# quanpn90/avsr

Measured on AMD Instinct MI355X. Metric: AV-frames/sec/GPU (fwd+bwd) on 15s clips; WER parity on LRS2 test, higher is better.
Workload: dtype bf16

## Files before the change

### avsr_amd/_lib.py

```python
import ctypes
import os

import torch

_HERE = os.path.dirname(os.path.abspath(__file__))
LIB_PATH = os.environ.get("AVSR_LIB_PATH_AB") or os.path.join(_HERE, "libavsr_hip.so")

AVSR_F32, AVSR_BF16 = 0, 1
ACT_NONE, ACT_GELU, ACT_RELU = 0, 1, 2

_c_p = ctypes.c_void_p
_i64 = ctypes.c_int64
_f = ctypes.c_float
_i = ctypes.c_int


class GemmParams(ctypes.Structure):
    _fields_ = [
        ("M", _i), ("N", _i), ("K", _i), ("batch", _i),
        ("dtype", _i), ("a_kmajor", _i), ("b_kmajor", _i), ("c_f32", _i),
        ("A", _c_p), ("lda", _i64), ("strideA", _i64),
        ("B", _c_p), ("ldb", _i64), ("strideB", _i64),
        ("C", _c_p), ("ldc", _i64), ("strideC", _i64),
        ("alpha", _f), ("beta", _f),
# ... 240 lines not shown
    _fields_ = [("B", _i), ("L", _i), ("x", _c_p), ("ldx", _i64), ("noise", _c_p), ("ldn", _i64),
                ("lengths", _c_p), ("snr_db", _c_p), ("y", _c_p), ("ldy", _i64), ("ws", _c_p)]


class VideoNormParams(ctypes.Structure):
    _fields_ = [
        ("B", _i), ("T", _i), ("H", _i), ("W", _i), ("crop", _i), ("oy", _i), ("ox", _i),
        ("frames", _c_p), ("mean", _f), ("std", _f), ("out", _c_p),
    ]


SYMBOLS = {
    "avsr_version": ([], ctypes.c_char_p),
    "avsr_set_option": ([_i, _i64], _i),
    "avsr_get_option": ([_i], _i64),
    "avsr_gemm": ([ctypes.POINTER(GemmParams), _c_p], _i),
    "avsr_gemm_wgrad_group": ([ctypes.POINTER(GemmParams), _i, _c_p], _i),
    "avsr_gemm_skinny_splits": ([_i, _i, _i], _i),
    "avsr_conv_fwd": ([ctypes.POINTER(ConvParams), _c_p], _i),
    "avsr_conv_bwd_data": ([ctypes.POINTER(ConvParams), _c_p], _i),
    "avsr_conv_bwd_weight": ([ctypes.POINTER(ConvParams), _c_p], _i),
    "avsr_conv_stat_tiles": ([ctypes.POINTER(ConvParams)], _i),
    "avsr_conv_bnr_tiles": ([ctypes.POINTER(ConvParams)], _i),
    "avsr_conv_wgrad_ws": ([ctypes.POINTER(ConvParams)], _i64),
    "avsr_conv_path": ([ctypes.POINTER(ConvParams), _i], _i),
    "avsr_layernorm_fwd": ([ctypes.POINTER(LayerNormParams), _c_p], _i),
    "avsr_layernorm_bwd": ([ctypes.POINTER(LayerNormParams), _c_p], _i),
    "avsr_bn_finalize": ([ctypes.POINTER(BnFinalizeParams), _c_p], _i),
    "avsr_bn_act_fwd": ([ctypes.POINTER(BnActParams), _c_p], _i),
    "avsr_bn_act_bwd_reduce": ([ctypes.POINTER(BnActParams), _c_p], _i),
    "avsr_bn_bwd_apply": ([ctypes.POINTER(BnActParams), _c_p], _i),
    "avsr_stem_pool_fwd": ([ctypes.POINTER(StemPoolParams), _c_p], _i),
    "avsr_stem_pool_bwd_apply": ([ctypes.POINTER(StemPoolParams), _c_p], _i),
    "avsr_bn_bwd_finalize": ([ctypes.POINTER(BnActParams), _i, _c_p], _i),
    "avsr_avgpool_fwd": ([_i, _i, _i, _i, _c_p, _c_p, _c_p], _i),
    "avsr_avgpool_bwd": ([_i, _i, _i, _i, _c_p, _c_p, _c_p], _i),
    "avsr_attn_fwd": ([ctypes.POINTER(AttnParams), _c_p], _i),
    "avsr_debug_attn_stamps": ([_c_p], _i),
    "avsr_attn_bwd_prep": ([ctypes.POINTER(AttnParams), _c_p], _i),
    "avsr_attn_bwd": ([ctypes.POINTER(AttnParams), _c_p], _i),
    "avsr_attn_dropmask": ([ctypes.POINTER(AttnParams), _c_p], _i),
    "avsr_attn_path": ([ctypes.POINTER(AttnParams), _i], _i),
    "avsr_row_lse": ([ctypes.POINTER(XentParams), _c_p], _i),
    "avsr_lsm_fwd": ([ctypes.POINTER(XentParams), _c_p], _i),
    "avsr_lsm_bwd": ([ctypes.POINTER(XentParams), _c_p], _i),
    "avsr_ctc_fwd": ([ctypes.POINTER(CtcParams), _c_p], _i),
    "avsr_ctc_bwd": ([ctypes.POINTER(CtcParams), _c_p], _i),
    "avsr_ctc_align": ([ctypes.POINTER(CtcAlignParams), _c_p], _i),
    "avsr_ctc_beam": ([ctypes.POINTER(CtcBeamParams), _c_p], _i),
    "avsr_loss_finalize": ([_i, _c_p, _i, _c_p, _c_p, _f, _i, _c_p, _c_p], _i),
    "avsr_ew_bwd": ([ctypes.POINTER(EwParams), _c_p], _i),
    "avsr_colsum_defer": ([_i], _i),
    "avsr_colsum_flush": ([_c_p], _i),
    "avsr_colsum_inline": ([_i], _i),
    "avsr_dropout_fwd": ([ctypes.POINTER(EwParams), _c_p], _i),
    "avsr_mask_rows": ([_i, _i, _i, _i, _c_p, _i64, _c_p, _c_p], _i),
    "avsr_embed_fwd": ([ctypes.POINTER(EmbedParams), _c_p], _i),
    "avsr_embed_bwd": ([ctypes.POINTER(EmbedParams), _c_p], _i),
    "avsr_cast": ([_i, _i, _i, _i, _c_p, _i64, _c_p, _i64, _f, _f, _c_p], _i),
    "avsr_cast_flat": ([_i, _i, _i64, _c_p, _c_p, _c_p], _i),
    "avsr_stem_pack": ([_i, _i, _i, _c_p, _c_p, _c_p], _i),
    "avsr_stem_wpack": ([_i, _c_p, _c_p, _c_p], _i),
    "avsr_stem_conv_tiles": ([_i, _i], _i),
    "avsr_stem_wpack2": ([_c_p, _c_p, _c_p], _i),
    "avsr_stem_conv_fwd": ([_i, _i, _c_p, _c_p, _c_p, _c_p, _c_p], _i),
    "avsr_stem_wgrad_unpack": ([_c_p, _c_p, _c_p], _i),
# ... 24 lines not shown
}

_lib = None


class AvsrLibError(RuntimeError):
    pass


def load():
    global _lib
    if _lib is not None:
        return _lib
    if not os.path.exists(LIB_PATH):
        raise AvsrLibError(f"{LIB_PATH} not built: run `python -c 'import __graft_entry__ as g; g.build()'`")
    lib = ctypes.CDLL(LIB_PATH, mode=ctypes.RTLD_GLOBAL)
    for name, (argtypes, restype) in SYMBOLS.items():
        if os.environ.get("AVSR_LIB_PATH_AB") and not hasattr(lib, name):
            continue
        fn = getattr(lib, name)
        fn.argtypes = argtypes
        fn.restype = restype
    _lib = lib
    return lib


def check(rc, op):
    if rc != 0:
        raise AvsrLibError(f"{op} failed with code {rc}")


OPTIONS = {"gemm_tile": 0, "attn_sq_fwd": 1, "attn_sq_bwd": 2, "wgrad_dual": 3, "conv_192": 4, "conv_s2phase": 5,
           "conv_patch": 6, "conv_wpatch": 7, "stem_pool_2x2": 8,
           "stem_wpatch": 9, "attn_enc_fused": 10}
TILES = ["128", "256", "256x128", "128x256", "128s3", "128w8s3", "pp", "192", "192x256", "192w8s3", "64", "64s4"]
ATTN_PATHS = ["f32", "tiled", "resident", "sq", "enc"]
CONV_PATHS = ["reg", "glds", "patch", "s2", "wpatch", "stem_wpatch"]
CONV_PASSES = ["fwd", "dgrad", "wgrad"]


def set_option(name, value):
    if name == "gemm_tile" and not isinstance(value, int):
        value = 0 if value in (None, "auto") else TILES.index(value) + 1
    lib = load()
    prev = get_option(name)
    check(lib.avsr_set_option(OPTIONS[name], int(value)), f"avsr_set_option({name}, {value})")
    return prev


def get_option(name):
    return int(load().avsr_get_option(OPTIONS[name]))


_raw_stream = getattr(torch._C, "_cuda_getCurrentRawStream", None)
_get_device = getattr(torch._C, "_cuda_getDevice", None) or torch.cuda.current_device


def stream_ptr(device=None):
    if _raw_stream is not None:
        idx = _get_device() if device is None else torch.device(device).index
        if idx is None:
            idx = _get_device()
        return ctypes.c_void_p(_raw_stream(idx))
    return ctypes.c_void_p(torch.cuda.current_stream(device).cuda_stream)
```

### avsr_amd/csrc/conv.h

```cpp
#pragma once
#include "gemm_core.h"
#include "gemm_glds.h"

namespace conv {
using namespace gemmcore;
using gemmg::GBK;
using gemmg::OOB;
using gemmg::bglds16;
using gemmg::make_rsrc;

struct ConvArgs {
  ConvGeom g;
  uint32_t a_bytes, b_bytes;
  const void* a; const void* b;
  int64_t a_gstride, b_gstride, c_gstride;
  int M, N, K, splits, kchunk;
  float* ws;
  Epi e;
  gemmg::BnrArgs bnr;
};

enum { K_FWD = 0, K_DGRAD = 1, K_WGRAD = 2, K_DGRAD_BNR = 3 };

struct WgradPlan { int splits, kchunk; bool slab; };
// ... 11 lines not shown

template <int R, int NW> struct BWgtR {
  static constexpr bool KMAJ = false;
  static constexpr int CPR = R / 8, RPP = 64 / CPR, SLOTS = GBK / RPP / NW;
  __amdgpu_buffer_rsrc_t rs; ConvGeom g;
  uint32_t vo[SLOTS];
  AVSR_DEV void init(const bf16* base, uint32_t bytes, const ConvGeom& g_, int r0, int rext, int wave, int lane) {
    rs = make_rsrc(base, bytes); g = g_;
    const int ktot = g.ktot_w;
#pragma unroll
    for (int i = 0; i < SLOTS; ++i) {
      const int pc = i * NW + wave, pk = pc * RPP + lane / CPR;
      const int r = r0 + ((lane % CPR) ^ gemmg::rswz<CPR>(pk)) * 8;
      vo[i] = r < rext ? (uint32_t)(((int64_t)pk * ktot + r) * 2) : OOB;
    }
  }
  AVSR_DEV void issue(char* img, int k0, int wave) const {
    const int ktot = g.ktot_w;
    int tap = k0 >> g.cout_shift;
    if (g.tap_step != 1) {
      const int u = (int)fdiv(tap, g.f_kw), v = tap - u * (int)g.f_kw.d;
      tap = (g.tap_kh0 + g.tap_step * u) * g.tap_kfw + g.tap_kw0 + g.tap_step * v;
    }
    const uint32_t so = (uint32_t)((((int64_t)(k0 & ((1 << g.cout_shift) - 1))) * ktot + (int64_t)tap * g.cin) * 2);
#pragma unroll
    for (int i = 0; i < SLOTS; ++i) bglds16(rs, vo[i], so, img + (i * NW + wave) * 1024);
  }
};

int igemm_f32(int kind, int bm, const ConvArgs& a, int groups, hipStream_t st);
int igemm_glds(int kind, int bm, const ConvArgs& a, int groups, hipStream_t st);
int patch_launch(int kind, const ConvArgs& a, const avsr_conv_params* p, hipStream_t st);
int wpatch_launch(const avsr_conv_params* p, hipStream_t st);
int stem_wpatch_launch(const avsr_conv_params* p, hipStream_t st);
int wgrad_reduce(float* ws, int splits, int chunks, int64_t mn, int groups, float* dw, int64_t dw_gstride, hipStream_t st);
}
```

### avsr_amd/csrc/conv.hip

```cpp
#include "conv.h"

namespace conv {
namespace {

int ilog2(int v) { int s = 0; while ((1 << s) < v) ++s; return (1 << s) == v ? s : -1; }

int make_geom(const avsr_conv_params* p, ConvGeom& g) {
  g.nimg = p->nimg; g.hin = p->hin; g.win = p->win; g.hout = p->hout; g.wout = p->wout;
  g.kh = p->kh; g.kw = p->kw; g.sh = p->sh; g.sw = p->sw; g.ph = p->ph; g.pw = p->pw;
  g.cin = p->cin; g.cout = p->cout; g.ldx = p->ldx; g.ldy = p->ldy;
  g.f_hw_out = make_fastdiv((uint32_t)(p->hout * p->wout));
  g.f_w_out = make_fastdiv((uint32_t)p->wout);
  g.f_hw_in = make_fastdiv((uint32_t)(p->hin * p->win));
  g.f_w_in = make_fastdiv((uint32_t)p->win);
  g.f_kw = make_fastdiv((uint32_t)p->kw);
  g.cin_shift = ilog2(p->cin); g.cout_shift = ilog2(p->cout);
  g.ktot_w = p->kh * p->kw * p->cin; g.tap_kfw = p->kw; g.tap_kh0 = 0; g.tap_kw0 = 0; g.tap_step = 1;
  const int ve = p->dtype == AVSR_BF16 ? 8 : 4;
  if (g.cin_shift < 0 || g.cout_shift < 0 || p->cin < ve || p->cout < ve) return AVSR_E_SHAPE;
  if (p->ldx % ve || p->ldy % ve) return AVSR_E_ALIGN;
  if (p->groups < 1 || p->ldx < (int64_t)p->groups * p->cin || p->ldy < (int64_t)p->groups * p->cout) return AVSR_E_SHAPE;
  return 0;
}

// ... 275 lines not shown
    a.bnr.scale = p->bnr_scale; a.bnr.shift = p->bnr_shift; a.bnr.prelu = p->bnr_prelu;
    a.bnr.mean = p->bnr_mean; a.bnr.invstd = p->bnr_invstd; a.bnr.scale2 = p->bnr_scale2;
    a.bnr.shift2 = p->bnr_shift2; a.bnr.mean2 = p->bnr_mean2; a.bnr.invstd2 = p->bnr_invstd2; a.bnr.ws = p->bnr_ws;
    kind = K_DGRAD_BNR + (p->bnr_scale2 ? 2 : p->bnr_res ? 1 : 0);
  }
  if (a.M == 0) return 0;
  ConvPlan pl;
  if ((rc = conv_plan(p, AVSR_CONV_DGRAD, pl))) return rc;
  a.a_bytes = pl.a_bytes; a.b_bytes = pl.b_bytes;
  hipStream_t st = (hipStream_t)stream;
  switch (pl.path) {
    case AVSR_CONV_PATH_REG: return igemm_f32(kind, pl.bm, a, p->groups, st);
    case AVSR_CONV_PATH_S2: return s2_launch(kind, a, p, pl, st);
    case AVSR_CONV_PATH_PATCH: return patch_launch(kind, a, p, st);
    default: return igemm_glds(kind, pl.bm, a, p->groups, st);
  }
}

extern "C" int avsr_conv_bwd_weight(const avsr_conv_params* p, void* stream) {
  if (!p) return AVSR_E_ARG;
  ConvArgs a{};
  int rc = make_geom(p, a.g);
  if (rc) return rc;
  if (!avsr_aligned16(p->x) || !avsr_aligned16(p->dy) || !p->dw) return AVSR_E_ALIGN;
  a.a = p->dy; a.b = p->x;
  const int64_t ktot = (int64_t)p->kh * p->kw * p->cin;
  a.a_gstride = p->cout; a.b_gstride = p->cin; a.c_gstride = p->cout * ktot;
  a.M = p->cout; a.N = (int)ktot; a.K = p->nimg * p->hout * p->wout;
  if (a.K == 0) return 0;
  ConvPlan pl;
  if ((rc = conv_plan(p, AVSR_CONV_WGRAD, pl))) return rc;
  hipStream_t st = (hipStream_t)stream;
  if (pl.path == AVSR_CONV_PATH_WPATCH) return wpatch_launch(p, st);
  if (pl.path == AVSR_CONV_PATH_STEM_WPATCH) return stem_wpatch_launch(p, st);
  const WgradPlan& w = pl.w;
  a.a_bytes = pl.a_bytes; a.b_bytes = pl.b_bytes;
  a.splits = w.splits; a.kchunk = w.kchunk;
  a.ws = w.slab ? p->ws : nullptr;
  a.e.M = a.M; a.e.N = a.N; a.e.C = p->dw; a.e.ldc = ktot; a.e.alpha = 1.f;
  if (w.slab) { a.e.ldc = a.N; }
  else if (w.splits == 1) { a.e.beta = 1.f; }
  else { a.e.atomic = 1; }
  rc = pl.path == AVSR_CONV_PATH_REG ? igemm_f32(K_WGRAD, pl.bm, a, p->groups, st) : igemm_glds(K_WGRAD, pl.bm, a, p->groups, st);
  if (rc || !w.slab) return rc;
  const int64_t mn = (int64_t)a.M * a.N;
  const int64_t xb = (int64_t)avsr_grid(mn / 4, 256, 1024) * p->groups;
  int chunks = (int)((65536 / 256 + xb - 1) / xb);
  if (chunks > w.splits) chunks = w.splits;
  if (chunks < 1) chunks = 1;
  return wgrad_reduce(p->ws, w.splits, chunks, mn, p->groups, p->dw, a.c_gstride, st);
}
```

### avsr_amd/csrc/conv_wpatch.hip

```cpp
#include "conv.h"

namespace conv {
namespace {

template <int W_, int TR_, int TPI_, int NBUF_, int PST_, int IPT_ = 1, int NBLK_ = WP_BLOCKS, int SPREAD_ = 0>
struct WPGeo {
  static constexpr int W = W_, TR = TR_, TPI = TPI_, H = TR * TPI, NBUF = NBUF_, PST = PST_, IPT = IPT_, NBLK = NBLK_;
  static constexpr int IMGT = TR * W;
  static constexpr int PX = IPT * IMGT;
  static constexpr int KS = (PX + 31) / 32;
  static constexpr int DYR = KS * 32;
  static constexpr int WP = W + 2, PROWS = (IPT * (TR + 1) + 1) * WP;
  static constexpr int SLOTS = PST / 16;
  static constexpr int PPIECE = (PROWS * SLOTS + 255) / 256;
  static constexpr int PBYTES = PPIECE * 4 * 1024;
  static constexpr int DYPIECE = DYR * 128 / 4096;
  static constexpr int DYB = DYR * 128;
  static constexpr int BUF = DYB + PBYTES;
  static constexpr int LDS = NBUF * BUF;
  static constexpr int NP = DYPIECE + PPIECE;
  static constexpr int SPREAD = SPREAD_ > 0 ? SPREAD_ : KS;
  static_assert(LDS <= 160 * 1024, "the tile buffers must fit the CU's LDS");
  static_assert(IPT == 1 || TPI == 1, "a tile is part of one image or whole images");
  static_assert(NBUF >= 2 && (NBUF - 2) * NP <= 63 && SPREAD <= KS, "vmcnt range / DMA spread");
// ... 186 lines not shown
}

template <class G>
int wpatch_launch_g(const avsr_conv_params* p, hipStream_t st) {
  static bool attr = false;
  if (!attr) {
    (void)hipFuncSetAttribute((const void*)conv_wgrad_patch_kernel<G>, hipFuncAttributeMaxDynamicSharedMemorySize, G::LDS);
    attr = true;
  }
  const uint32_t bytes = (uint32_t)((int64_t)p->nimg * p->hin * p->win * p->cin * 2);
  const int nq = (p->cout / 64) * (p->cin / 64), S = G::NBLK / 8;
  if (nq <= S ? S % nq != 0 : (nq % S != 0 || 8 % (nq / S) != 0)) return AVSR_E_SHAPE;
  hipLaunchKernelGGL((conv_wgrad_patch_kernel<G>), dim3(G::NBLK), dim3(256), G::LDS, st, (const bf16*)p->x,
                     (const bf16*)p->dy, bytes, bytes, p->nimg, p->cin, p->cout, p->ws);
  AVSR_CHECK_LAUNCH();
  const unsigned gx = (64 * WP_COLS / 4 + 255) / 256;
  hipLaunchKernelGGL(wpatch_reduce_kernel, dim3(gx, (unsigned)nq, (unsigned)WPR_CHUNKS), dim3(256), 0, st, p->ws,
                     G::NBLK, p->cin, p->cout, p->dw, 0);
  AVSR_CHECK_LAUNCH();
  hipLaunchKernelGGL(wpatch_reduce_kernel, dim3(gx, (unsigned)nq, 1u), dim3(256), 0, st, p->ws, G::NBLK, p->cin,
                     p->cout, p->dw, 1);
  AVSR_CHECK_LAUNCH();
  return 0;
}

constexpr int SWP_TR = 4, SWP_TC = 48, SWP_KS = SWP_TC / 8, SWP_TPI = 44 / SWP_TR;
constexpr int SWP_DYB = SWP_KS * 32 * 128, SWP_DYPIECE = SWP_DYB / 4096;
constexpr int SWP_PR = 2 * SWP_TR + 5, SWP_PC = 103, SWP_SLOTS = SWP_PR * SWP_PC, SWP_RB = SWP_PC * 16;
constexpr int SWP_PPIECE = (SWP_SLOTS + 255) / 256, SWP_PBYTES = SWP_PPIECE * 4096;
constexpr int SWP_BUF = SWP_DYB + SWP_PBYTES, SWP_NBUF = 3, SWP_LDS = SWP_NBUF * SWP_BUF;
constexpr int SWP_NP = SWP_DYPIECE + SWP_PPIECE, SWP_PAIRS = 25;
constexpr int SWP_JW = (SWP_PAIRS + 3) / 4;
static_assert(SWP_LDS <= 160 * 1024 && SWP_DYB % 4096 == 0 && SWP_KS % 2 == 0, "stem weight-grad tile buffers");
static_assert(2 * (SWP_TC - 1) + 6 - 3 < SWP_PC - 3 + 1 && SWP_NP % SWP_KS == 0, "patch width / DMA spread");

AVSR_DEV int swp_toff(int t) {
  t = t > 48 ? 48 : t;
  const int kh = t / 7, kw = t - 7 * kh;
  return kh * SWP_RB + kw * 16;
}

__global__ __launch_bounds__(256, 1) void stem_wgrad_patch_kernel(const bf16* __restrict__ xp, const bf16* __restrict__ dy,
                                                                  uint32_t x_bytes, uint32_t dy_bytes, int nimg,
                                                                  float* __restrict__ ws) {
  extern __shared__ __attribute__((aligned(16))) char smem[];
  const int lane = threadIdx.x & 63, wave = __builtin_amdgcn_readfirstlane(threadIdx.x >> 6);
  const int ntiles = nimg * SWP_TPI;
  const int ta = (int)((int64_t)ntiles * blockIdx.x / gridDim.x), tb = (int)((int64_t)ntiles * (blockIdx.x + 1) / gridDim.x);
  const __amdgpu_buffer_rsrc_t rx = make_rsrc(xp, x_bytes), rdy = make_rsrc(dy, dy_bytes);
  uint32_t vdy[SWP_DYPIECE];
  int vpt[SWP_PPIECE], ppr[SWP_PPIECE];
#pragma unroll
  for (int i = 0; i < SWP_DYPIECE; ++i) {
    const int sl = (wave + 4 * i) * 64 + lane, row = sl >> 3;
    const int ch = (sl & 7) ^ whswz(row), k = row & 31, col = 8 * (row >> 5) + (k & 7);
    vdy[i] = col < 44 ? (uint32_t)(((k >> 3) * 44 + col) * 128 + ch * 16) : gemmg::OOB;
  }
#pragma unroll
  for (int i = 0; i < SWP_PPIECE; ++i) {
    const int sl = (wave + 4 * i) * 64 + lane, pr = sl / SWP_PC, pc = sl - pr * SWP_PC;
    const bool ok = sl < SWP_SLOTS && pc >= 3 && pc < 91;
    vpt[i] = ((pr - 3) * 88 + pc - 3) * 16;
    ppr[i] = ok ? pr - 3 : -1000;
  }
  auto issue = [&](int pc, int t, char* buf) {
    const int img = t / SWP_TPI, oy0 = (t - img * SWP_TPI) * SWP_TR;
    if (pc < SWP_DYPIECE) {
      gemmg::bglds16(rdy, vdy[pc], (uint32_t)(img * 1936 + oy0 * 44) * 128u, buf + (wave + 4 * pc) * 1024);
    } else {
      const int i = pc - SWP_DYPIECE, y = 2 * oy0 + ppr[i];
      const uint32_t vo = (uint32_t)y < 88u ? (uint32_t)(img * 123904 + oy0 * 2816 + vpt[i]) : gemmg::OOB;
      gemmg::bglds16(rx, vo, 0u, buf + SWP_DYB + (wave + 4 * i) * 1024);
    }
  };
  const int g = lane >> 4, qq = (lane & 15) >> 2, pp = lane & 3;
  const int pxa = 16 * (g >> 1) + 4 * (g & 1) + qq;
  const int sw = whswz(pxa);
  int dA[4];
#pragma unroll
  for (int i = 0; i < 4; ++i) dA[i] = pxa * 128 + (((2 * i + (pp >> 1)) ^ sw) << 4) + 8 * (pp & 1);
  const int pbase = SWP_DYB + (2 * (pxa >> 3) * SWP_PC + 2 * (pxa & 7)) * 16;
  int oB[SWP_JW];
#pragma unroll
  for (int j = 0; j < SWP_JW; ++j) oB[j] = pbase + swp_toff(2 * (wave + 4 * j) + (pp >> 1)) + 8 * (pp & 1);
  f32x4 acc[4][SWP_JW];
#pragma unroll
  for (int i = 0; i < 4; ++i)
#pragma unroll
    for (int j = 0; j < SWP_JW; ++j) acc[i][j] = f32x4{0.f, 0.f, 0.f, 0.f};
  constexpr int PD = SWP_NBUF - 1, PER = SWP_NP / SWP_KS;
#pragma unroll
  for (int d = 0; d < PD; ++d)
    if (ta + d < tb)
#pragma unroll
      for (int pc = 0; pc < SWP_NP; ++pc) issue(pc, ta + d, smem + d * SWP_BUF);
  struct Fr { bf16x8 a[4], b[SWP_JW]; };
  auto load = [&](Fr& f, const char* buf, int kb) {
#pragma unroll
    for (int i = 0; i < 4; ++i) f.a[i] = trpair(buf + dA[i] + kb * 4096, buf + dA[i] + kb * 4096 + 1024);
#pragma unroll
    for (int j = 0; j < SWP_JW; ++j) f.b[j] = trpair(buf + oB[j] + kb * 256, buf + oB[j] + kb * 256 + 2 * SWP_RB);
  };
  auto mma = [&](const Fr& f, int h) {
#pragma unroll
    for (int i = 2 * h; i < 2 * h + 2; ++i)
#pragma unroll
      for (int j = 0; j < SWP_JW; ++j) acc[i][j] = mfma16(f.a[i], f.b[j], acc[i][j]);
  };
  for (int t = ta; t < tb; ++t) {
    const char* buf = smem + ((t - ta) % SWP_NBUF) * SWP_BUF;
    char* nbuf = smem + ((t + PD - ta) % SWP_NBUF) * SWP_BUF;
    const bool more = t + PD < tb;
    if (t + 1 < tb) gemmg::wait_vmcnt<SWP_NP>();
    else gemmg::wait_vmcnt<0>();
    __builtin_amdgcn_s_barrier();
    asm volatile("" ::: "memory");
    Fr f0, f1;
    load(f0, buf, 0);
#pragma unroll
    for (int kb = 0; kb < SWP_KS; kb += 2) {
      mma(f0, 0);
      __builtin_amdgcn_sched_barrier(0);
      load(f1, buf, kb + 1);
      __builtin_amdgcn_sched_barrier(0);
      mma(f0, 1);
      if (more)
#pragma unroll
        for (int d = 0; d < PER; ++d) issue(kb * PER + d, t + PD, nbuf);
      mma(f1, 0);
      __builtin_amdgcn_sched_barrier(0);
      if (kb + 2 < SWP_KS) load(f0, buf, kb + 2);
      __builtin_amdgcn_sched_barrier(0);
      mma(f1, 1);
      if (more)
#pragma unroll
        for (int d = 0; d < PER; ++d) issue((kb + 1) * PER + d, t + PD, nbuf);
    }
  }
  float* o = ws + (int64_t)blockIdx.x * 64 * SWP_COLS;
#pragma unroll
  for (int j = 0; j < SWP_JW; ++j) {
    const int col = 16 * (wave + 4 * j) + (lane & 15);
    if (col < SWP_COLS)
#pragma unroll
      for (int i = 0; i < 4; ++i)
#pragma unroll
        for (int r = 0; r < 4; ++r) o[(16 * i + 4 * g + r) * SWP_COLS + col] = acc[i][j][r];
  }
}

}

int wpatch_launch(const avsr_conv_params* p, hipStream_t st) {
  if (p->cin == 64) return wpatch_launch_g<WPStage1>(p, st);
  if (p->cin == 128) return wpatch_launch_g<WPStage2>(p, st);
  if (p->cin == 256) return wpatch_launch_g<WPStage3>(p, st);
  return wpatch_launch_g<WPStage4>(p, st);
}

int stem_wpatch_launch(const avsr_conv_params* p, hipStream_t st) {
  static bool attr = false;
  if (!attr) {
    (void)hipFuncSetAttribute((const void*)stem_wgrad_patch_kernel, hipFuncAttributeMaxDynamicSharedMemorySize, SWP_LDS);
    attr = true;
  }
  const uint32_t xb = (uint32_t)((int64_t)p->nimg * 88 * 88 * 16), dyb = (uint32_t)((int64_t)p->nimg * 1936 * 128);
  hipLaunchKernelGGL(stem_wgrad_patch_kernel, dim3(SWP_BLOCKS), dim3(256), SWP_LDS, st, (const bf16*)p->x,
                     (const bf16*)p->dy, xb, dyb, p->nimg, p->ws);
  AVSR_CHECK_LAUNCH();
  return wgrad_reduce(p->ws, SWP_BLOCKS, 8, 64 * SWP_COLS, 1, p->dw, 0, st);
}
}
```

### avsr_amd/csrc/version.hip

```cpp
#include <atomic>

#include "common.h"

extern "C" const char* avsr_version(void) { return "avsr_hip 0.2.0 gfx950"; }

#ifndef AVSR_AB_ATTN_ENC_FUSED
#define AVSR_AB_ATTN_ENC_FUSED 1
#endif

namespace {
std::atomic<int64_t> g_opt[AVSR_OPT_COUNT] = {{0}, {1}, {0}, {1}, {1}, {1}, {1}, {1}, {1}, {1}, {AVSR_AB_ATTN_ENC_FUSED}};

bool opt_valid(int option, int64_t v) {
  switch (option) {
    case AVSR_OPT_GEMM_TILE: return v >= 0 && v <= AVSR_TILE_COUNT;
    case AVSR_OPT_ATTN_SQ_BWD: return v == 0;
    case AVSR_OPT_ATTN_SQ_FWD:
    case AVSR_OPT_WGRAD_DUAL:
    case AVSR_OPT_CONV_192:
    case AVSR_OPT_CONV_S2PHASE:
    case AVSR_OPT_CONV_PATCH:
    case AVSR_OPT_CONV_WPATCH:
    case AVSR_OPT_STEM_POOL_2X2:
    case AVSR_OPT_STEM_WPATCH:
    case AVSR_OPT_ATTN_ENC_FUSED: return v == 0 || v == 1;
    default: return false;
  }
}
}

int64_t avsr_opt(int option) { return g_opt[option].load(std::memory_order_relaxed); }

extern "C" int avsr_set_option(int option, int64_t value) {
  if (!opt_valid(option, value)) return AVSR_E_ARG;
  g_opt[option].store(value, std::memory_order_relaxed);
  return 0;
}

extern "C" int64_t avsr_get_option(int option) {
  if (option < 0 || option >= AVSR_OPT_COUNT) return -1;
  return avsr_opt(option);
}
```

### avsr_amd/engine.py

```python
import math
import os
import random

import numpy as np
import torch

from . import ops
from . import _lib as L
from .arena import Arena

GELU, RELU, NONE = L.ACT_GELU, L.ACT_RELU, L.ACT_NONE
_BN_FUSE = True
_DB_FUSE = True
_COLSUM_DEFER = True
_SIDE_BIAS = True
WGRAD_GROUP = False
SIDE_ORDER = "o,f2,f1,c,q"
ATTN_MASK = True
_CTC_SIDE = True
_STEM_DIRECT = True
_LN_EW_FUSE = True
SIDE_STREAM = True
EARLY_NORM = True
OPT_OVERLAP = True
# ... 544 lines not shown
                dz1, sums1 = da1, ops.bn_bwd_finalize(ws, tiles, cout, **g1)
            else:
                ops.conv_bwd_data(blk["g2"], dh2, self.w(p + "conv2.weight"), da1)
                dz1, sums1 = ops.bn_act_bwd_reduce(da1, blk["h1"], blk["st1"], prelu1, **g1)
            dh1 = self._e(M2, cout)
            ops.bn_bwd_apply(dz1, blk["h1"], blk["st1"], sums1, dh1)
            if self._live(p + "conv1.weight"):
                self._conv_wgrad(blk["g1"], blk["x"], dh1, self.g(p + "conv1.weight"))
            if fuse:
                if j > 0:
                    pb = blocks[j - 1]
                    pdown = pb["gd"] is not None
                    tgt = dict(h=pb["h2"], st=pb["st2"], prelu=self.arena.master(pb["p"] + "relu2.weight"),
                               res=pb["hd"] if pdown else pb["x"], st2=pb["std"] if pdown else None)
                else:
                    tgt = dict(h=ctx["hmax"], st=ctx["st0"], prelu=self.arena.master(R + "frontend3D.2.weight"))
            red = None
            if not down:
                dx = dz2
                if fuse:
                    red = ops.conv_bwd_data_bnr(blk["g1"], dh1, self.w(p + "conv1.weight"), dx, beta=1.0, **tgt)
                else:
                    ops.conv_bwd_data(blk["g1"], dh1, self.w(p + "conv1.weight"), dx, beta=1.0)
            else:
                dx = self._e(blk["x"].shape[0], cin)
                ops.conv_bwd_data(blk["g1"], dh1, self.w(p + "conv1.weight"), dx)
                if self._live(p + "downsample.0.weight"):
                    self._conv_wgrad(blk["gd"], blk["x"], dhd, self.g(p + "downsample.0.weight"))
                if fuse:
                    red = ops.conv_bwd_data_bnr(blk["gd"], dhd, self.w(p + "downsample.0.weight"), dx, beta=1.0, **tgt)
                else:
                    ops.conv_bwd_data(blk["gd"], dhd, self.w(p + "downsample.0.weight"), dx, beta=1.0)
            dout = dx
        dh0 = self._e(N * 44 * 44, 64)
        dzp, sums = ops.stem_pool_bwd_reduce(dout, ctx["hmax"], N, 44, 44, ctx["st0"],
                                             self.arena.master(R + "frontend3D.2.weight"),
                                             dprelu=self.g(R + "frontend3D.2.weight"),
                                             dgamma=self.g(R + "frontend3D.1.weight"),
                                             dbeta=self.g(R + "frontend3D.1.bias"), reduced=red)
        ops.stem_pool_bwd_apply(dzp, ctx["am"], ctx["h0"], N, 44, 44, ctx["st0"], sums, dh0)
        if self._live(R + "frontend3D.0.weight"):
            gp = self._z(64, 7, 7, 8, dtype=torch.float32)
            ops.conv_bwd_weight(ctx["gs"], ctx["xp"], dh0, gp)
            ops.stem_wgrad_unpack(gp, self.g(R + "frontend3D.0.weight"))

    def _ln(self, x, name, eps, save=None):
        y, mean, rstd = ops.layernorm_fwd(x, self.arena.master(name + ".weight"), self.arena.master(name + ".bias"), eps)
        return y, mean, rstd

    def _ln_bwd(self, dy, x, name, mean, rstd, dres=None, dx=None, ew=None):
        if ew is not None and _LN_EW_FUSE:
            g, p, seed, dbn = ew
            return ops.layernorm_bwd(dy, x, self.arena.master(name + ".weight"), mean, rstd, dx=dx, dres=dres,
                                     dgamma=self.g(name + ".weight"), dbeta=self.g(name + ".bias"), g=g, drop_p=p,
                                     seed=seed, db=self.g(dbn))
        out = ops.layernorm_bwd(dy, x, self.arena.master(name + ".weight"), mean, rstd, dx=dx, dres=dres,
                                dgamma=self.g(name + ".weight"), dbeta=self.g(name + ".bias"))
        if ew is not None:
            g, p, seed, dbn = ew
            ops.ew_bwd(out, out=g, drop_p=p, seed=seed, db=self.g(dbn))
        return out

    def encoder_fwd(self, audios, videos, bt, train, save, seeds, modality=None, plan=None):
        cfg = self.cfg
        B, T = bt["B"], bt["T"]
        M, D = B * T, self.D
        EN = "encoder."
        cut = 0 if plan is None else plan.cut
        ctx = {"B": B, "T": T, "modality": modality, "plan": plan}
        draws = [float(torch.rand([])) for _ in range(self.nl)]
        kept = [i for i in range(self.nl) if not (train and draws[i] < self.layerdrop)]
        p_att = cfg.attention_dropout if train else 0.0
        amask = self._attn_masks(B, T, p_att, {i: seeds.peek(3 + 4 * j) for j, i in enumerate(kept)})
        add = self.fuse_add
        fcat = self._e(M, D if add else 2 * D)
        fa = self._e(M, D) if add else fcat[:, :D]
# ... 595 lines not shown
```

### avsr_amd/ops.py

```python
import ctypes
import os

import torch

from . import _lib as L

_DT = {torch.float32: L.AVSR_F32, torch.bfloat16: L.AVSR_BF16}

PROBE = {}

SLAB_PAD = 1088


def slab_ws(batch, splitk, M, N):
    return batch * splitk * (M * N + SLAB_PAD)


def dtype_code(t):
    try:
        return _DT[t.dtype]
    except KeyError:
        raise L.AvsrLibError(f"unsupported dtype {t.dtype}")


# ... 416 lines not shown
    C = h.shape[-1]
    _call("avsr_stem_pool_fwd", L.fill(L.StemPoolParams, dtype=dtype_code(h), nimg=nimg, H=H, W=W, C=C,
                                        Ho=(H + 1) // 2, Wo=(W + 1) // 2, h=h, scale=st.scale, shift=st.shift,
                                        prelu=prelu, y=y, argmax=argmax, hmax=hmax))
    return y


def stem_pool_bwd(dy, argmax, hmax, h, nimg, H, W, st, prelu, dh, *, dzp=None, sums=None, dprelu=None,
                  dgamma=None, dbeta=None, reduced=None):
    dzp, sums = stem_pool_bwd_reduce(dy, hmax, nimg, H, W, st, prelu, dzp=dzp, sums=sums, dprelu=dprelu,
                                     dgamma=dgamma, dbeta=dbeta, reduced=reduced)
    return stem_pool_bwd_apply(dzp, argmax, h, nimg, H, W, st, sums, dh)


def stem_pool_bwd_reduce(dy, hmax, nimg, H, W, st, prelu, *, dzp=None, sums=None, dprelu=None, dgamma=None,
                         dbeta=None, reduced=None):
    C = hmax.shape[-1]
    Mo = nimg * ((H + 1) // 2) * ((W + 1) // 2)
    if reduced is None:
        return bn_act_bwd_reduce(dy.view(Mo, C), hmax.view(Mo, C), st, prelu, dz=dzp, sums=sums,
                                 dprelu=dprelu, dgamma=dgamma, dbeta=dbeta)
    return dy, bn_bwd_finalize(reduced[0], reduced[1], C, sums=sums, dprelu=dprelu, dgamma=dgamma, dbeta=dbeta)


def stem_pool_bwd_apply(dzp, argmax, h, nimg, H, W, st, sums, dh, m_total=0):
    C = h.shape[-1]
    _call("avsr_stem_pool_bwd_apply", L.fill(L.StemPoolParams, dtype=dtype_code(h), nimg=nimg, H=H, W=W, C=C,
                                              Ho=(H + 1) // 2, Wo=(W + 1) // 2, h=h, scale=st.scale, argmax=argmax,
                                              dz=dzp, mean=st.mean, invstd=st.invstd, sums=sums, dh=dh,
                                              m_total=int(m_total)))
    return dh


def avgpool_fwd(x, nimg, P, C, y):
    L.check(L.load().avsr_avgpool_fwd(dtype_code(x), nimg, P, C, x.data_ptr(), y.data_ptr(), L.stream_ptr()),
            "avsr_avgpool_fwd")
    return y


def avgpool_bwd(dy, nimg, P, C, dx):
    L.check(L.load().avsr_avgpool_bwd(dtype_code(dy), nimg, P, C, dy.data_ptr(), dx.data_ptr(), L.stream_ptr()),
            "avsr_avgpool_bwd")
    return dx



def _attn_params(q, k, v, o, B, H, Lq, Lk, lse, klen, causal, scale, drop_p, seed):
    return L.fill(L.AttnParams, dtype=dtype_code(q), B=B, H=H, Lq=Lq, Lk=Lk, scale=scale,
                  q=q, ldq=q.stride(0), k=k, ldk=k.stride(0), v=v, ldv=v.stride(0), o=o, ldo=o.stride(0),
                  lse=lse, klen=klen, causal=int(causal), drop_p=float(drop_p), seed=int(seed) & (2 ** 64 - 1))


def attn_path(dtype, B, H, Lq, Lk, *, causal=False, backward=False, ld=None, lddo=None):
    ld = H * 64 if ld is None else ld
    p = L.fill(L.AttnParams, dtype=_DT.get(dtype, dtype), B=B, H=H, Lq=Lq, Lk=Lk, causal=int(causal), ldq=ld, ldk=ld,
               ldv=ld, ldo=ld, lddo=H * 64 if lddo is None else lddo)
    rc = L.load().avsr_attn_path(ctypes.byref(p), int(backward))
    if not 0 <= rc < len(L.ATTN_PATHS):
        L.check(rc, "avsr_attn_path")
    return L.ATTN_PATHS[rc]


def attn_mask_words(B, H, Lq, Lk):
    return B * H * ((Lq + 31) // 32) * (2 * ((Lk + 63) // 64)) * 16


# ... 447 lines not shown
```

### include/avsr_hip.h

```cpp
#ifndef AVSR_HIP_H
#define AVSR_HIP_H

#include <stdint.h>

#ifdef __cplusplus
extern "C" {
#endif

enum { AVSR_F32 = 0, AVSR_BF16 = 1 };
enum { AVSR_ACT_NONE = 0, AVSR_ACT_GELU = 1, AVSR_ACT_RELU = 2 };
enum { AVSR_E_SHAPE = 1001, AVSR_E_ALIGN = 1002, AVSR_E_DTYPE = 1003, AVSR_E_ARG = 1004 };

const char* avsr_version(void);

enum {
  AVSR_OPT_GEMM_TILE = 0,
  AVSR_OPT_ATTN_SQ_FWD = 1,
  AVSR_OPT_ATTN_SQ_BWD = 2,
  AVSR_OPT_WGRAD_DUAL = 3,
  AVSR_OPT_CONV_192 = 4,
  AVSR_OPT_CONV_S2PHASE = 5,
  AVSR_OPT_CONV_PATCH = 6,
  AVSR_OPT_CONV_WPATCH = 7,
  AVSR_OPT_STEM_POOL_2X2 = 8,
  AVSR_OPT_STEM_WPATCH = 9,
  AVSR_OPT_ATTN_ENC_FUSED = 10,
  AVSR_OPT_COUNT = 11
};
enum {
  AVSR_TILE_128 = 0, AVSR_TILE_256 = 1, AVSR_TILE_256x128 = 2, AVSR_TILE_128x256 = 3, AVSR_TILE_128s3 = 4,
  AVSR_TILE_128w8s3 = 5, AVSR_TILE_PP = 6, AVSR_TILE_192 = 7, AVSR_TILE_192x256 = 8, AVSR_TILE_192w8s3 = 9,
  AVSR_TILE_64 = 10, AVSR_TILE_64s4 = 11, AVSR_TILE_COUNT = 12
};
int avsr_set_option(int option, int64_t value);
int64_t avsr_get_option(int option);

typedef struct {
  int M, N, K, batch;
  int dtype;
  int a_kmajor, b_kmajor;
  int c_f32;
  const void* A; int64_t lda, strideA;
  const void* B; int64_t ldb, strideB;
  void* C;       int64_t ldc, strideC;
  float alpha, beta;
  const float* bias;
  int act;
  int epi_bwd;
  void* preact;
  const void* res;  int64_t ldr, strideR;
  const void* gate;
  float drop_p;
  uint64_t seed;
  int splitk;
  float* ws;
  float* db;
  float* db_ws;
  unsigned long long* stamp;
  float* skinny_ws;
  const float* ln_c1;
// ... 90 lines not shown
  const float* scale2; const float* shift2;
  const float* prelu;
  void* y;
  const void* dy; void* dz;
  const float* mean; const float* invstd;
  const float* mean2; const float* invstd2;
  float* sums;
  float* dprelu;
  float* dgamma; float* dbeta; float* dgamma2; float* dbeta2;
  void* dh; void* dh2; float beta_acc;
  float* ws;
} avsr_bn_act_params;
#define AVSR_BN_FIN_WS(tiles, C) (((int64_t)(tiles) + ((tiles) > 256 ? ((tiles) + 15) / 16 : 0)) * 4 * (C))
#define AVSR_BN_WS(C) AVSR_BN_FIN_WS(2048, C)
int avsr_bn_act_fwd(const avsr_bn_act_params* p, void* stream);
int avsr_bn_act_bwd_reduce(const avsr_bn_act_params* p, void* stream);
int avsr_bn_bwd_finalize(const avsr_bn_act_params* p, int tiles, void* stream);
int avsr_bn_bwd_apply(const avsr_bn_act_params* p, void* stream);

typedef struct {
  int dtype, nimg, H, W, C, Ho, Wo;
  const void* h; const float* scale; const float* shift; const float* prelu;
  void* y; uint8_t* argmax;
  const void* dy; void* dz;
  const float* mean; const float* invstd;
  float* sums; float* dprelu; float* dgamma; float* dbeta;
  float* ws;
  void* hmax;
  void* dh;
  int64_t m_total;
} avsr_stem_pool_params;
int avsr_stem_pool_fwd(const avsr_stem_pool_params* p, void* stream);
int avsr_stem_pool_bwd_apply(const avsr_stem_pool_params* p, void* stream);

int avsr_avgpool_fwd(int dtype, int nimg, int P, int C, const void* x, void* y, void* stream);
int avsr_avgpool_bwd(int dtype, int nimg, int P, int C, const void* dy, void* dx, void* stream);

typedef struct {
  int dtype, B, H, Lq, Lk;
  float scale;
  const void* q; int64_t ldq;
  const void* k; int64_t ldk;
  const void* v; int64_t ldv;
  void* o; int64_t ldo;
  float* lse;
  const int* klen;
  int causal;
  float drop_p; uint64_t seed;
  const void* dout; int64_t lddo;
  float* delta;
  float* dq; int64_t lddq;
  void* dk; int64_t lddk;
  void* dv; int64_t lddv;
  void* dq_out; int64_t lddq_out;
  float* db; float* db_ws;
  uint64_t* drop_mask;
} avsr_attn_params;
#define AVSR_ATTN_DB_WS(B, H) ((int64_t)(B) * 3 * (H) * 64)
#define AVSR_ATTN_MASK_WORDS(B, H, Lq, Lk) \
  ((int64_t)(B) * (H) * (((Lq) + 31) / 32) * (2 * (((Lk) + 63) / 64)) * 16)
int avsr_debug_attn_stamps(unsigned long long* buf);
int avsr_attn_fwd(const avsr_attn_params* p, void* stream);
int avsr_attn_bwd_prep(const avsr_attn_params* p, void* stream);
int avsr_attn_bwd(const avsr_attn_params* p, void* stream);
enum { AVSR_ATTN_FWD = 0, AVSR_ATTN_BWD = 1 };
enum {
// ... 288 lines not shown
```

Measured before the change: 147,600.

## Fuse stem pool backward apply into stem weight-grad patch kernel via producer waves

Measured after the change: 147,500, median of 4. About the same (-0.0%).

```diff
diff --git a/avsr_amd/_lib.py b/avsr_amd/_lib.py
--- a/avsr_amd/_lib.py
+++ b/avsr_amd/_lib.py
@@ -296,6 +296,8 @@
     "avsr_bn_bwd_apply": ([ctypes.POINTER(BnActParams), _c_p], _i),
     "avsr_stem_pool_fwd": ([ctypes.POINTER(StemPoolParams), _c_p], _i),
     "avsr_stem_pool_bwd_apply": ([ctypes.POINTER(StemPoolParams), _c_p], _i),
+    "avsr_stem_bwd_wgrad_fused": ([ctypes.POINTER(StemPoolParams), ctypes.POINTER(ConvParams)], _i),
+    "avsr_stem_bwd_wgrad": ([ctypes.POINTER(StemPoolParams), ctypes.POINTER(ConvParams), _c_p], _i),
     "avsr_bn_bwd_finalize": ([ctypes.POINTER(BnActParams), _i, _c_p], _i),
     "avsr_avgpool_fwd": ([_i, _i, _i, _i, _c_p, _c_p, _c_p], _i),
     "avsr_avgpool_bwd": ([_i, _i, _i, _i, _c_p, _c_p, _c_p], _i),
@@ -386,7 +388,7 @@
 
 OPTIONS = {"gemm_tile": 0, "attn_sq_fwd": 1, "attn_sq_bwd": 2, "wgrad_dual": 3, "conv_192": 4, "conv_s2phase": 5,
            "conv_patch": 6, "conv_wpatch": 7, "stem_pool_2x2": 8,
-           "stem_wpatch": 9, "attn_enc_fused": 10}
+           "stem_wpatch": 9, "attn_enc_fused": 10, "stem_bwd_fused": 11}
 TILES = ["128", "256", "256x128", "128x256", "128s3", "128w8s3", "pp", "192", "192x256", "192w8s3", "64", "64s4"]
 ATTN_PATHS = ["f32", "tiled", "resident", "sq", "enc"]
 CONV_PATHS = ["reg", "glds", "patch", "s2", "wpatch", "stem_wpatch"]
diff --git a/avsr_amd/csrc/conv.h b/avsr_amd/csrc/conv.h
--- a/avsr_amd/csrc/conv.h
+++ b/avsr_amd/csrc/conv.h
@@ -67,6 +67,6 @@
 int igemm_glds(int kind, int bm, const ConvArgs& a, int groups, hipStream_t st);
 int patch_launch(int kind, const ConvArgs& a, const avsr_conv_params* p, hipStream_t st);
 int wpatch_launch(const avsr_conv_params* p, hipStream_t st);
-int stem_wpatch_launch(const avsr_conv_params* p, hipStream_t st);
+int stem_wpatch_launch(const avsr_conv_params* p, const avsr_stem_pool_params* sp, hipStream_t st);
 int wgrad_reduce(float* ws, int splits, int chunks, int64_t mn, int groups, float* dw, int64_t dw_gstride, hipStream_t st);
 }
diff --git a/avsr_amd/csrc/conv.hip b/avsr_amd/csrc/conv.hip
--- a/avsr_amd/csrc/conv.hip
+++ b/avsr_amd/csrc/conv.hip
@@ -331,7 +331,7 @@
   if ((rc = conv_plan(p, AVSR_CONV_WGRAD, pl))) return rc;
   hipStream_t st = (hipStream_t)stream;
   if (pl.path == AVSR_CONV_PATH_WPATCH) return wpatch_launch(p, st);
-  if (pl.path == AVSR_CONV_PATH_STEM_WPATCH) return stem_wpatch_launch(p, st);
+  if (pl.path == AVSR_CONV_PATH_STEM_WPATCH) return stem_wpatch_launch(p, nullptr, st);
   const WgradPlan& w = pl.w;
   a.a_bytes = pl.a_bytes; a.b_bytes = pl.b_bytes;
   a.splits = w.splits; a.kchunk = w.kchunk;
@@ -349,3 +349,29 @@
   if (chunks < 1) chunks = 1;
   return wgrad_reduce(p->ws, w.splits, chunks, mn, p->groups, p->dw, a.c_gstride, st);
 }
+
+extern "C" int avsr_stem_bwd_wgrad_fused(const avsr_stem_pool_params* sp, const avsr_conv_params* p) {
+  if (!sp || !p || !avsr_opt(AVSR_OPT_STEM_BWD_FUSED) || sp->dtype != AVSR_BF16 || p->dtype != AVSR_BF16) return 0;
+  if (sp->H != 44 || sp->W != 44 || sp->C != 64 || sp->Ho != 22 || sp->Wo != 22 || sp->nimg != p->nimg || sp->nimg <= 0) return 0;
+  ConvGeom g;
+  ConvPlan pl;
+  return make_geom(p, g) == 0 && conv_plan(p, AVSR_CONV_WGRAD, pl) == 0 && pl.path == AVSR_CONV_PATH_STEM_WPATCH;
+}
+
+extern "C" int avsr_stem_bwd_wgrad(const avsr_stem_pool_params* sp, const avsr_conv_params* p, void* stream) {
+  if (!sp || !p) return AVSR_E_ARG;
+  if (sp->dtype != AVSR_BF16 && sp->dtype != AVSR_F32) return AVSR_E_DTYPE;
+  if (sp->dtype != p->dtype) return AVSR_E_ARG;
+  if (avsr_stem_bwd_wgrad_fused(sp, p)) {
+    if (!sp->dz || !sp->argmax || !sp->h || !sp->sums || !sp->scale || !sp->mean || !sp->invstd) return AVSR_E_ARG;
+    if (!avsr_aligned16(p->x) || !avsr_aligned16(sp->h) || !avsr_aligned16(sp->dz) || ((uintptr_t)sp->argmax & 7) || !p->dw)
+      return AVSR_E_ALIGN;
+    return stem_wpatch_launch(p, sp, (hipStream_t)stream);
+  }
+  if (!sp->dh) return AVSR_E_SHAPE;
+  const int rc = avsr_stem_pool_bwd_apply(sp, stream);
+  if (rc) return rc;
+  avsr_conv_params q = *p;
+  q.dy = sp->dh;
+  return avsr_conv_bwd_weight(&q, stream);
+}
diff --git a/avsr_amd/csrc/conv_wpatch.hip b/avsr_amd/csrc/conv_wpatch.hip
--- a/avsr_amd/csrc/conv_wpatch.hip
+++ b/avsr_amd/csrc/conv_wpatch.hip
@@ -242,7 +242,8 @@
 constexpr int SWP_NP = SWP_DYPIECE + SWP_PPIECE, SWP_PAIRS = 25;
 constexpr int SWP_JW = (SWP_PAIRS + 3) / 4;
 static_assert(SWP_LDS <= 160 * 1024 && SWP_DYB % 4096 == 0 && SWP_KS % 2 == 0, "stem weight-grad tile buffers");
-static_assert(2 * (SWP_TC - 1) + 6 - 3 < SWP_PC - 3 + 1 && SWP_NP % SWP_KS == 0, "patch width / DMA spread");
+static_assert(2 * (SWP_TC - 1) + 6 - 3 < SWP_PC - 3 + 1 && SWP_NP % SWP_KS == 0 && SWP_PPIECE % SWP_KS == 0,
+              "patch width / DMA spread");
 
 AVSR_DEV int swp_toff(int t) {
   t = t > 48 ? 48 : t;
@@ -250,13 +251,121 @@
   return kh * SWP_RB + kw * 16;
 }
 
-__global__ __launch_bounds__(256, 1) void stem_wgrad_patch_kernel(const bf16* __restrict__ xp, const bf16* __restrict__ dy,
-                                                                  uint32_t x_bytes, uint32_t dy_bytes, int nimg,
-                                                                  float* __restrict__ ws) {
+struct StemApply {
+  const bf16* h; const bf16* dz; const uint8_t* am;
+  const float* scale; const float* mean; const float* invstd; const float* sums;
+  int64_t m_total;
+};
+
+struct SwpRaw { bf16x8 h[4], g[4]; uint2 am[4]; };
+
+template <int NB>
+AVSR_DEV void swp_produce(const StemApply& ap, int nimg, int ta, int tb, char* smem, int pt) {
+  const int cg = pt & 7, slot = pt >> 3;
+  const float invM = 1.f / (ap.m_total > 0 ? (float)ap.m_total : (float)nimg * 44 * 44);
+  float ka[8], kb[8], kc[8], km[8];
+#pragma unroll
+  for (int j = 0; j < 8; ++j) {
+    const int c = cg * 8 + j;
+    const float s0 = ap.sums[c * 3 + 0] * invM, s1 = ap.sums[c * 3 + 1] * invM;
+    ka[j] = ap.scale[c]; kb[j] = -ap.scale[c] * s1 * ap.invstd[c]; kc[j] = -ap.scale[c] * s0; km[j] = ap.mean[c];
+  }
+  auto place = [&](int u, int& br, int& bc) {
+    const int b = slot + 32 * u;
+    br = b >= 22 ? 1 : 0;
+    bc = b < 44 ? b - 22 * br : 0;
+    return b < 44;
+  };
+  auto fetch = [&](SwpRaw& R, int t, int u) {
+    int br, bc;
+    place(u, br, bc);
+    const int img = t / SWP_TPI, oh = (t - img * SWP_TPI) * (SWP_TR / 2) + br, ow = bc;
+#pragma unroll
+    for (int w = 0; w < 4; ++w) {
+      const int64_t ov = ((img * 22 + min(oh + (w >> 1), 21)) * 22 + min(ow + (w & 1), 21)) * 8 + cg;
+      R.g[w] = *(const bf16x8*)(ap.dz + ov * 8);
+      R.am[w] = *(const uint2*)(ap.am + ov * 8);
+    }
+    const int64_t hb = ((img * 44 + 2 * oh) * 44 + 2 * ow) * 8 + cg;
+#pragma unroll
+    for (int qd = 0; qd < 4; ++qd) R.h[qd] = *(const bf16x8*)(ap.h + (hb + ((qd >> 1) * 44 + (qd & 1)) * 8) * 8);
+  };
+  auto emit = [&](const SwpRaw& R, int t, int u, char* buf) {
+    int br, bc;
+    if (!place(u, br, bc)) return;
+    const int oh = (t % SWP_TPI) * (SWP_TR / 2) + br, ow = bc;
+    bool wok[4];
+    uint8_t am[4][8];
+#pragma unroll
+    for (int w = 0; w < 4; ++w) {
+      wok[w] = oh + (w >> 1) < 22 && ow + (w & 1) < 22;
+      *(uint2*)am[w] = R.am[w];
+    }
+#pragma unroll
+    for (int qd = 0; qd < 4; ++qd) {
+      const int dy = qd >> 1, dx = qd & 1;
+      float d[8];
+#pragma unroll
+      for (int j = 0; j < 8; ++j) d[j] = 0.f;
+#pragma unroll
+      for (int w = 0; w < 4; ++w) {
+        const int wa = w >> 1, wb = w & 1;
+        if ((wa && !dy) || (wb && !dx)) continue;
+        const uint8_t want = (uint8_t)((dy - 2 * wa + 1) * 3 + (dx - 2 * wb + 1));
+#pragma unroll
+        for (int j = 0; j < 8; ++j) d[j] += (wok[w] && am[w][j] == want) ? (float)R.g[w][j] : 0.f;
+      }
+      bf16x8 o;
+#pragma unroll
+      for (int j = 0; j < 8; ++j)
+        o[j] = (bf16)(__builtin_fmaf(ka[j], d[j], kb[j] * ((float)R.h[qd][j] - km[j])) + kc[j]);
+      const int r = 2 * br + dy, col = 2 * bc + dx, row = (col >> 3) * 32 + r * 8 + (col & 7);
+      *(bf16x8*)(buf + row * 128 + ((cg ^ whswz(row)) << 4)) = o;
+    }
+  };
+  for (int v = pt; v < SWP_NBUF * 128; v += 256) {
+    const int row = 5 * 32 + ((v >> 5) & 3) * 8 + 4 + ((v >> 3) & 3);
+    *(uint4*)(smem + (v >> 7) * SWP_BUF + row * 128 + (v & 7) * 16) = uint4{0u, 0u, 0u, 0u};
+  }
+  SwpRaw R[3];
+  fetch(R[0], ta, 0);
+  fetch(R[1], min(ta + 1 / NB, tb - 1), 1 % NB);
+  for (int t0 = ta; t0 < tb; t0 += 3) {
+#pragma unroll
+    for (int p = 0; p < 3; ++p) {
+      const int t = t0 + p;
+      if (t >= tb) break;
+      char* buf = smem + ((t - ta) % SWP_NBUF) * SWP_BUF;
+#pragma unroll
+      for (int u = 0; u < NB; ++u) {
+        const int k = p * NB + u;
+        fetch(R[(k + 2) % 3], min(t + (u + 2) / NB, tb - 1), (u + 2) % NB);
+        emit(R[k % 3], t, u, buf);
+      }
+      asm volatile("s_waitcnt lgkmcnt(0)" ::: "memory");
+      __builtin_amdgcn_s_barrier();
+    }
+  }
+}
+
+template <bool FUSED>
+__global__ __launch_bounds__(FUSED ? 512 : 256, 1) void stem_wgrad_patch_kernel(const bf16* __restrict__ xp,
+                                                                                const bf16* __restrict__ dy, uint32_t x_bytes,
+                                                                                uint32_t dy_bytes, int nimg,
+                                                                                float* __restrict__ ws, StemApply ap) {
   extern __shared__ __attribute__((aligned(16))) char smem[];
   const int lane = threadIdx.x & 63, wave = __builtin_amdgcn_readfirstlane(threadIdx.x >> 6);
   const int ntiles = nimg * SWP_TPI;
   const int ta = (int)((int64_t)ntiles * blockIdx.x / gridDim.x), tb = (int)((int64_t)ntiles * (blockIdx.x + 1) / gridDim.x);
+  if constexpr (FUSED) {
+    if (wave >= 4) {
+      if (ta == tb) return;
+      if (wave < 6) swp_produce<2>(ap, nimg, ta, tb, smem, (int)threadIdx.x - 256);
+      else swp_produce<1>(ap, nimg, ta, tb, smem, (int)threadIdx.x - 256);
+      return;
+    }
+  }
+  constexpr int DYP = FUSED ? 0 : SWP_DYPIECE, NP = DYP + SWP_PPIECE;
   const __amdgpu_buffer_rsrc_t rx = make_rsrc(xp, x_bytes), rdy = make_rsrc(dy, dy_bytes);
   uint32_t vdy[SWP_DYPIECE];
   int vpt[SWP_PPIECE], ppr[SWP_PPIECE];
@@ -275,11 +384,18 @@
   }
   auto issue = [&](int pc, int t, char* buf) {
     const int img = t / SWP_TPI, oy0 = (t - img * SWP_TPI) * SWP_TR;
-    if (pc < SWP_DYPIECE) {
+    if (pc < DYP) {
       gemmg::bglds16(rdy, vdy[pc], (uint32_t)(img * 1936 + oy0 * 44) * 128u, buf + (wave + 4 * pc) * 1024);
     } else {
-      const int i = pc - SWP_DYPIECE, y = 2 * oy0 + ppr[i];
-      const uint32_t vo = (uint32_t)y < 88u ? (uint32_t)(img * 123904 + oy0 * 2816 + vpt[i]) : gemmg::OOB;
+      const int i = pc - DYP;
+      int vp = vpt[i], pr = ppr[i];
+      if constexpr (FUSED) {
+        const int sl = (wave + 4 * i) * 64 + lane, r = sl / SWP_PC, c = sl - r * SWP_PC;
+        vp = ((r - 3) * 88 + c - 3) * 16;
+        pr = sl < SWP_SLOTS && c >= 3 && c < 91 ? r - 3 : -1000;
+      }
+      const int y = 2 * oy0 + pr;
+      const uint32_t vo = (uint32_t)y < 88u ? (uint32_t)(img * 123904 + oy0 * 2816 + vp) : gemmg::OOB;
       gemmg::bglds16(rx, vo, 0u, buf + SWP_DYB + (wave + 4 * i) * 1024);
     }
   };
@@ -298,12 +414,12 @@
   for (int i = 0; i < 4; ++i)
 #pragma unroll
     for (int j = 0; j < SWP_JW; ++j) acc[i][j] = f32x4{0.f, 0.f, 0.f, 0.f};
-  constexpr int PD = SWP_NBUF - 1, PER = SWP_NP / SWP_KS;
+  constexpr int PD = SWP_NBUF - 1, PER = NP / SWP_KS;
 #pragma unroll
   for (int d = 0; d < PD; ++d)
     if (ta + d < tb)
 #pragma unroll
-      for (int pc = 0; pc < SWP_NP; ++pc) issue(pc, ta + d, smem + d * SWP_BUF);
+      for (int pc = 0; pc < NP; ++pc) issue(pc, ta + d, smem + d * SWP_BUF);
   struct Fr { bf16x8 a[4], b[SWP_JW]; };
   auto load = [&](Fr& f, const char* buf, int kb) {
 #pragma unroll
@@ -321,7 +437,7 @@
     const char* buf = smem + ((t - ta) % SWP_NBUF) * SWP_BUF;
     char* nbuf = smem + ((t + PD - ta) % SWP_NBUF) * SWP_BUF;
     const bool more = t + PD < tb;
-    if (t + 1 < tb) gemmg::wait_vmcnt<SWP_NP>();
+    if (t + 1 < tb) gemmg::wait_vmcnt<NP>();
     else gemmg::wait_vmcnt<0>();
     __builtin_amdgcn_s_barrier();
     asm volatile("" ::: "memory");
@@ -368,15 +484,22 @@
   return wpatch_launch_g<WPStage4>(p, st);
 }
 
-int stem_wpatch_launch(const avsr_conv_params* p, hipStream_t st) {
+int stem_wpatch_launch(const avsr_conv_params* p, const avsr_stem_pool_params* sp, hipStream_t st) {
   static bool attr = false;
   if (!attr) {
-    (void)hipFuncSetAttribute((const void*)stem_wgrad_patch_kernel, hipFuncAttributeMaxDynamicSharedMemorySize, SWP_LDS);
+    (void)hipFuncSetAttribute((const void*)stem_wgrad_patch_kernel<false>, hipFuncAttributeMaxDynamicSharedMemorySize, SWP_LDS);
+    (void)hipFuncSetAttribute((const void*)stem_wgrad_patch_kernel<true>, hipFuncAttributeMaxDynamicSharedMemorySize, SWP_LDS);
     attr = true;
   }
   const uint32_t xb = (uint32_t)((int64_t)p->nimg * 88 * 88 * 16), dyb = (uint32_t)((int64_t)p->nimg * 1936 * 128);
-  hipLaunchKernelGGL(stem_wgrad_patch_kernel, dim3(SWP_BLOCKS), dim3(256), SWP_LDS, st, (const bf16*)p->x,
-                     (const bf16*)p->dy, xb, dyb, p->nimg, p->ws);
+  if (sp) {
+    const StemApply ap{(const bf16*)sp->h, (const bf16*)sp->dz, sp->argmax, sp->scale, sp->mean, sp->invstd, sp->sums, sp->m_total};
+    hipLaunchKernelGGL(stem_wgrad_patch_kernel<true>, dim3(SWP_BLOCKS), dim3(512), SWP_LDS, st, (const bf16*)p->x,
+                       (const bf16*)nullptr, xb, 0u, p->nimg, p->ws, ap);
+  } else {
+    hipLaunchKernelGGL(stem_wgrad_patch_kernel<false>, dim3(SWP_BLOCKS), dim3(256), SWP_LDS, st, (const bf16*)p->x,
+                       (const bf16*)p->dy, xb, dyb, p->nimg, p->ws, StemApply{});
+  }
   AVSR_CHECK_LAUNCH();
   return wgrad_reduce(p->ws, SWP_BLOCKS, 8, 64 * SWP_COLS, 1, p->dw, 0, st);
 }
diff --git a/avsr_amd/csrc/version.hip b/avsr_amd/csrc/version.hip
--- a/avsr_amd/csrc/version.hip
+++ b/avsr_amd/csrc/version.hip
@@ -7,9 +7,13 @@
 #ifndef AVSR_AB_ATTN_ENC_FUSED
 #define AVSR_AB_ATTN_ENC_FUSED 1
 #endif
+#ifndef AVSR_AB_STEM_BWD_FUSED
+#define AVSR_AB_STEM_BWD_FUSED 1
+#endif
 
 namespace {
-std::atomic<int64_t> g_opt[AVSR_OPT_COUNT] = {{0}, {1}, {0}, {1}, {1}, {1}, {1}, {1}, {1}, {1}, {AVSR_AB_ATTN_ENC_FUSED}};
+std::atomic<int64_t> g_opt[AVSR_OPT_COUNT] = {{0}, {1}, {0}, {1}, {1}, {1}, {1}, {1}, {1}, {1}, {AVSR_AB_ATTN_ENC_FUSED},
+                                              {AVSR_AB_STEM_BWD_FUSED}};
 
 bool opt_valid(int option, int64_t v) {
   switch (option) {
@@ -23,7 +27,8 @@
     case AVSR_OPT_CONV_WPATCH:
     case AVSR_OPT_STEM_POOL_2X2:
     case AVSR_OPT_STEM_WPATCH:
-    case AVSR_OPT_ATTN_ENC_FUSED: return v == 0 || v == 1;
+    case AVSR_OPT_ATTN_ENC_FUSED:
+    case AVSR_OPT_STEM_BWD_FUSED: return v == 0 || v == 1;
     default: return false;
   }
 }
diff --git a/avsr_amd/engine.py b/avsr_amd/engine.py
--- a/avsr_amd/engine.py
+++ b/avsr_amd/engine.py
@@ -600,16 +600,19 @@
                 else:
                     ops.conv_bwd_data(blk["gd"], dhd, self.w(p + "downsample.0.weight"), dx, beta=1.0)
             dout = dx
-        dh0 = self._e(N * 44 * 44, 64)
         dzp, sums = ops.stem_pool_bwd_reduce(dout, ctx["hmax"], N, 44, 44, ctx["st0"],
                                              self.arena.master(R + "frontend3D.2.weight"),
                                              dprelu=self.g(R + "frontend3D.2.weight"),
                                              dgamma=self.g(R + "frontend3D.1.weight"),
                                              dbeta=self.g(R + "frontend3D.1.bias"), reduced=red)
-        ops.stem_pool_bwd_apply(dzp, ctx["am"], ctx["h0"], N, 44, 44, ctx["st0"], sums, dh0)
         if self._live(R + "frontend3D.0.weight"):
             gp = self._z(64, 7, 7, 8, dtype=torch.float32)
-            ops.conv_bwd_weight(ctx["gs"], ctx["xp"], dh0, gp)
+            if ops.stem_bwd_fused(ctx["gs"], ctx["xp"], ctx["h0"], N, 44, 44):
+                ops.stem_bwd_wgrad(ctx["gs"], ctx["xp"], dzp, ctx["am"], ctx["h0"], N, 44, 44, ctx["st0"], sums, gp)
+            else:
+                dh0 = self._e(N * 44 * 44, 64)
+                ops.stem_pool_bwd_apply(dzp, ctx["am"], ctx["h0"], N, 44, 44, ctx["st0"], sums, dh0)
+                ops.conv_bwd_weight(ctx["gs"], ctx["xp"], dh0, gp)
             ops.stem_wgrad_unpack(gp, self.g(R + "frontend3D.0.weight"))
 
     def _ln(self, x, name, eps, save=None):
diff --git a/avsr_amd/ops.py b/avsr_amd/ops.py
--- a/avsr_amd/ops.py
+++ b/avsr_amd/ops.py
@@ -472,6 +472,33 @@
     return dh
 
 
+def _stem_bwd_wgrad_params(g, x, dzp, argmax, h, nimg, H, W, st, sums, dw, dh, m_total):
+    sp = L.fill(L.StemPoolParams, dtype=dtype_code(h), nimg=nimg, H=H, W=W, C=h.shape[-1], Ho=(H + 1) // 2,
+                Wo=(W + 1) // 2, h=h, scale=st and st.scale, argmax=argmax, dz=dzp, mean=st and st.mean,
+                invstd=st and st.invstd, sums=sums, dh=dh, m_total=int(m_total))
+    p = g.params(dtype_code(x))
+    p.x = x.data_ptr()
+    p.dw = 0 if dw is None else dw.data_ptr()
+    p.ws = 1
+    return sp, p
+
+
+def stem_bwd_fused(g, x, h, nimg, H, W):
+    sp, p = _stem_bwd_wgrad_params(g, x, None, None, h, nimg, H, W, None, None, None, None, 0)
+    return bool(L.load().avsr_stem_bwd_wgrad_fused(ctypes.byref(sp), ctypes.byref(p)))
+
+
+def stem_bwd_wgrad(g, x, dzp, argmax, h, nimg, H, W, st, sums, dw, dh=None, m_total=0):
+    assert x.dtype == h.dtype and dw.dtype == torch.float32
+    sp, p = _stem_bwd_wgrad_params(g, x, dzp, argmax, h, nimg, H, W, st, sums, dw, dh, m_total)
+    lib = L.load()
+    n = lib.avsr_conv_wgrad_ws(ctypes.byref(p))
+    ws = torch.empty(max(n, 1), device=dw.device, dtype=torch.float32)
+    p.ws = ws.data_ptr() if n > 0 else 0
+    L.check(lib.avsr_stem_bwd_wgrad(ctypes.byref(sp), ctypes.byref(p), L.stream_ptr()), "avsr_stem_bwd_wgrad")
+    return dw
+
+
 def avgpool_fwd(x, nimg, P, C, y):
     L.check(L.load().avsr_avgpool_fwd(dtype_code(x), nimg, P, C, x.data_ptr(), y.data_ptr(), L.stream_ptr()),
             "avsr_avgpool_fwd")
diff --git a/include/avsr_hip.h b/include/avsr_hip.h
--- a/include/avsr_hip.h
+++ b/include/avsr_hip.h
@@ -25,7 +25,8 @@
   AVSR_OPT_STEM_POOL_2X2 = 8,
   AVSR_OPT_STEM_WPATCH = 9,
   AVSR_OPT_ATTN_ENC_FUSED = 10,
-  AVSR_OPT_COUNT = 11
+  AVSR_OPT_STEM_BWD_FUSED = 11,
+  AVSR_OPT_COUNT = 12
 };
 enum {
   AVSR_TILE_128 = 0, AVSR_TILE_256 = 1, AVSR_TILE_256x128 = 2, AVSR_TILE_128x256 = 3, AVSR_TILE_128s3 = 4,
@@ -182,6 +183,8 @@
 } avsr_stem_pool_params;
 int avsr_stem_pool_fwd(const avsr_stem_pool_params* p, void* stream);
 int avsr_stem_pool_bwd_apply(const avsr_stem_pool_params* p, void* stream);
+int avsr_stem_bwd_wgrad_fused(const avsr_stem_pool_params* sp, const avsr_conv_params* c);
+int avsr_stem_bwd_wgrad(const avsr_stem_pool_params* sp, const avsr_conv_params* c, void* stream);
 
 int avsr_avgpool_fwd(int dtype, int nimg, int P, int C, const void* x, void* y, void* stream);
 int avsr_avgpool_bwd(int dtype, int nimg, int P, int C, const void* dy, void* dx, void* stream);
```
